# lab-incert/peba1

Hardware: AMD Instinct MI355X
Metric: bootstrapped gates/sec (blind rotations/s) over the PEBA1 match path, and end-to-end match ms (higher is better)
Workload: dtype u32

## Files before the change

include/tfhe_hip.h:

```cpp
#ifndef TFHE_HIP_H
#define TFHE_HIP_H

#include "tfhe/tfhe_core.h"

#ifdef __cplusplus
extern "C" {
#endif

enum TfheHipGate {
    TFHE_HIP_NAND = 0, TFHE_HIP_OR, TFHE_HIP_AND, TFHE_HIP_NOR, TFHE_HIP_XOR, TFHE_HIP_XNOR,
    TFHE_HIP_ANDNY, TFHE_HIP_ANDYN, TFHE_HIP_ORNY, TFHE_HIP_ORYN
};

const char *tfhe_hip_last_error(void);
void tfhe_hip_clear_error(void);

int tfhe_hip_set_device(int device);
int tfhe_hip_get_device(void);
int tfhe_hip_device_pci_bus_id(char *out, int len);

TFheGateBootstrappingParameterSet *tfhe_hip_new_parameters(
    int32_t n, int32_t N, int32_t k, int32_t l, int32_t Bgbit, int32_t ks_t, int32_t ks_basebit,
    double ks_stdev, double bk_stdev, double max_stdev);
TFheGateBootstrappingParameterSet *tfhe_hip_new_p2048_parameters(void);
// ... 103 lines not shown
    uint64_t clk_ref_ticks;
    uint64_t dead_gates;
    uint64_t folded_gates;
    uint64_t br_wide4_launches;
    uint64_t br_split_launches;
    uint64_t br_wave8_launches;
    uint64_t br_wave2_launches;
    uint64_t br_tables0_launches;
    uint64_t br_tables1_launches;
    uint64_t br_tables2_launches;
    uint64_t lut_rotations;
    uint64_t multi_rotations;
    uint64_t multi_outputs;
    uint64_t lincomb_ops;
    uint64_t lincomb_launches;
} TfheHipStats;
void tfhe_hip_get_stats(TfheHipStats *out);
void tfhe_hip_reset_stats(void);
void tfhe_hip_set_kernel_timing(int on);
int tfhe_hip_last_flush_keys(void);
int tfhe_hip_set_batch_keys(int on);

int tfhe_hip_test_form_admissible(int form, int32_t N, int32_t l, int32_t Bgbit, int tables);

void tfhe_hip_test_set_alloc_cap(int64_t bytes);

int tfhe_hip_test_schedule(const int32_t *ops5, int32_t count, int32_t unit, int32_t balance, int32_t *levels_out);
int tfhe_hip_test_level_plan(const int32_t *ops5, const int32_t *op_keys, int32_t count, int32_t nkeys, int32_t unit,
                             int32_t balance, int32_t *levels_out, int32_t *sizes6, int32_t *rot_off, int32_t *ks_off,
                             int32_t *rot_koff, int32_t *ks_koff, int32_t *rot_key, int32_t *rots6, int32_t *kss4);
// ... 2 lines not shown
                              int32_t *rot_koff, int32_t *ks_koff, int32_t *rot_key, int32_t *rots8, int32_t *kss4);
int tfhe_hip_test_level_plan_lut(const int32_t *ops10, const int32_t *op_keys, int32_t count, int32_t nkeys, int32_t unit,
                                 int32_t balance, int32_t reuse, int32_t *levels_out, int32_t *shared_with, int32_t *sizes6,
                                 int32_t *rot_off, int32_t *ks_off, int32_t *rot_koff, int32_t *ks_koff, int32_t *rot_key,
                                 int32_t *rots9, int32_t *kss4);
int tfhe_hip_test_level_plan_multi(const int32_t *ops16, const int32_t *op_keys, int32_t count, int32_t nkeys, int32_t unit,
                                   int32_t balance, int32_t reuse, const int32_t *dead_slots, int32_t ndead,
                                   int32_t *levels_out, int32_t *shared_with, int32_t *sizes6, int32_t *rot_off, int32_t *ks_off,
                                   int32_t *rot_koff, int32_t *ks_koff, int32_t *rot_key, int32_t *rots10, int32_t *kss4);
int tfhe_hip_test_level_plan_lin(const int32_t *ops16, const int32_t *op_keys, int32_t count, int32_t nkeys, int32_t unit,
                                 int32_t balance, int32_t reuse, const int32_t *dead_slots, int32_t ndead,
                                 const int32_t *lin_terms2, int32_t nterms, int32_t *levels_out, int32_t *ranks_out,
                                 int32_t *shared_with, int32_t *sizes6, int32_t *rot_off, int32_t *ks_off, int32_t *rot_koff,
                                 int32_t *ks_koff, int32_t *rot_key, int32_t *rots10, int32_t *kss4, int32_t *lin_sizes2,
                                 int32_t *lin_level_off, int32_t *lin_launch_off, int32_t *lin_launch_rank, int32_t *lins35);
int tfhe_hip_test_br_plan(int32_t N, int32_t l, int32_t Bgbit, const int32_t *tunings4, int32_t cu_count, int32_t count,
                          int32_t flags, int32_t *out3);
int tfhe_hip_test_ks_plan(int32_t n, int32_t N, int32_t k, int32_t ks_t, int32_t ks_basebit, const int32_t *tunings5,
                          int32_t cu_count, int32_t count, int64_t *out6);
int tfhe_hip_test_wg_times(const TFheGateBootstrappingCloudKeySet *bk, int32_t width, uint64_t *times4, double *launch_ms);

int tfhe_hip_kernel_negacyclic(const TFheGateBootstrappingCloudKeySet *bk, const int32_t *ip,
                               const Torus32 *tp, Torus32 *res, int32_t count);
int tfhe_hip_kernel_bootstrap_woks(const TFheGateBootstrappingCloudKeySet *bk, const Torus32 *lin,
                                   int32_t count, Torus32 *u_out, Torus32 *acc_out);
int tfhe_hip_kernel_lut_bootstrap_woks(const TFheGateBootstrappingCloudKeySet *bk, const Torus32 *lin, int32_t count,
                                       const int32_t *lut_index, const Torus32 *polys, int32_t npolys, Torus32 *u_out,
                                       Torus32 *acc_out);
#define TFHE_HIP_EXTRACT_SPEC_WORDS 73
int tfhe_hip_kernel_lut_bootstrap_multi_woks(const TFheGateBootstrappingCloudKeySet *bk, const Torus32 *lin, int32_t count,
// ... 11 lines not shown
```

peba1_amd/api.py:

```python
import ctypes as C

import numpy as np

from . import lib as _l

GATE_CODES = {"NAND": 0, "OR": 1, "AND": 2, "NOR": 3, "XOR": 4, "XNOR": 5,
              "ANDNY": 6, "ANDYN": 7, "ORNY": 8, "ORYN": 9}
GATE3_CODES = {"MAJ3": 0, "XOR3": 1, "XNOR3": 2}
GATE3_LIN = {"MAJ3": 1, "XOR3": -2, "XNOR3": 2}


def _i32p(a):
    assert a.dtype == np.int32 and a.flags["C_CONTIGUOUS"]
    return a.ctypes.data_as(_l.I32P)


def last_error():
    return _l.load().tfhe_hip_last_error().decode()


class _CFile:
    _libc = None

    def __init__(self, path, mode):
# ... 398 lines not shown

def flush_async():
    return _l.load().tfhe_hip_flush_async()


def wait():
    return _l.load().tfhe_hip_wait()


def set_tuning(name, value):
    if _l.load().tfhe_hip_set_tuning(name.encode(), int(value)) != 0:
        raise ValueError(last_error())


def stats():
    s = _l.StatsAll()
    _l.load().tfhe_hip_get_stats(C.byref(s))
    return {f: getattr(s, f) for f in _l.STATS_FIELDS}


def last_flush_keys():
    return _l.load().tfhe_hip_last_flush_keys()


def reset_stats():
    _l.load().tfhe_hip_reset_stats()


def kernel_negacyclic(key, ip, tp):
    ip = np.ascontiguousarray(ip, dtype=np.int32)
    tp = np.ascontiguousarray(tp, dtype=np.int32)
    res = np.zeros_like(tp)
    rc = _l.load().tfhe_hip_kernel_negacyclic(key.cloud, _i32p(ip), _i32p(tp), _i32p(res), ip.shape[0])
# ... 73 lines not shown
```

peba1_amd/csrc/engine.cpp:

```cpp
#include "engine.hpp"

#include <algorithm>
#include <utility>
#include <vector>
#include <chrono>
#include <ctime>
#include <unistd.h>
#include <cstdio>
#include <cstdlib>
#include <cstring>
#include <mutex>

#include "br_forms.hpp"
#include "ntt_field.hpp"

namespace tfhe_hip {

static std::string g_last_error;
static std::mutex g_err_mtx;

void set_error(const std::string &msg) {
    std::lock_guard<std::mutex> g(g_err_mtx);
    g_last_error = msg;
}
// ... 73 lines not shown
    for (size_t i = new_cap; i-- > cap_;) free_.push_back((int32_t)i);
    cap_ = new_cap;
}
int32_t SlotPool::alloc() {
    if (free_.empty()) {
        if (cap_ >= max_cap_)
            api_fail("ciphertext slot pool exhausted (" + std::to_string(max_cap_) +
                     " slots); raise TFHE_HIP_POOL_SLOTS or free ciphertext arrays");
        grow(std::min(max_cap_, cap_ * 2));
    }
    const int32_t s = free_.back();
    free_.pop_back();
    ref_[s] = 1;
    level[s] = 0;
    pending[s] = 0;
    return s;
}
void SlotPool::release(int32_t s) {
    if (s < 0) return;
    if (--ref_[s] == 0) free_.push_back(s);
}

Engine &Engine::get() {
    static Engine e;
    return e;
}

void Engine::set_device(int d) {
    if (inited_.load() && d != device_) fatal("tfhe_hip_set_device after the engine was initialised");
    device_ = d;
// ... 316 lines not shown
    if (n_ring < 1 || n_ring > LUT_STRIDE) api_fail("a test polynomial of more than " + std::to_string(LUT_STRIDE) + " words");
    return g_luts.add(pad_rows(words, 1, (size_t)n_ring, LUT_STRIDE).data());
}
void Engine::lut_free(int32_t index) { g_luts.release(index); }

int32_t Engine::spec_add(const ExtractSpec &xs) {
    ENGINE_DEVICE_SCOPE();
    ensure_init();
    if (g_specs.free.empty() && g_specs.used == g_specs.cap && g_specs.cap > (size_t)XS_ENTRY_MASK / 2) api_fail("too many extract specs");
    const int32_t index = g_specs.add(&xs);
    if (spec_nout_.size() <= (size_t)index) spec_nout_.resize((size_t)index + 1, 0);
    spec_nout_[(size_t)index] = xs.nout;
    return index;
}
void Engine::spec_free(int32_t index) { g_specs.release(index); }

SlotPool *Engine::find_pool(const Params &p) const {
    for (SlotPool *pl : pools_)
        if (pl->ct_stride() == p.ct_stride() && pl->ct_words() == p.ct_words()) return pl;
    return nullptr;
}

SlotPool *Engine::pool_for(const Params &p) {
    ENGINE_DEVICE_SCOPE();
    ensure_init();
    if (SlotPool *pl = find_pool(p)) return pl;
    size_t cap = 1u << 22;
    if (const char *env = std::getenv("TFHE_HIP_POOL_SLOTS")) cap = (size_t)std::atoll(env);
    if (cap < 8 || cap > MAX_POOL_SLOTS) {
        set_error("TFHE_HIP_POOL_SLOTS out of range [8, 2^29]; clamped");
// ... 539 lines not shown
```

peba1_amd/csrc/engine.hpp:

```cpp
#pragma once
#include <hip/hip_runtime.h>

#include <atomic>
#include <chrono>
#include <cstdint>
#include <string>
#include <vector>

#include "host_keys.hpp"
#include "br_forms.hpp"
#include "launch_plan.hpp"
#include "kernels.hpp"
#include "../../include/tfhe_hip.h"

struct DeviceKeyImage {
    tfhe_hip::DevParams dp;
    tfhe_hip::DevKey key;
    bool form_ok[tfhe_hip::BR_FORM_COUNT][3] = {};
    uint32_t *bk_img = nullptr;
    int32_t *ksk = nullptr;
    uint32_t *tw = nullptr;
    size_t bk_img_bytes = 0, ksk_bytes = 0, tw_bytes = 0;
};

// ... 13 lines not shown

class SlotPool {
public:
    SlotPool(int ct_words, int ct_stride, size_t capacity);
    ~SlotPool();
    int32_t alloc();
    void retain(int32_t s) { ++ref_[s]; }
    int32_t refs(int32_t s) const { return ref_[s]; }
    void release(int32_t s);
    int32_t *data() { return data_; }
    int ct_stride() const { return stride_; }
    int ct_words() const { return words_; }
    size_t capacity() const { return max_cap_; }
    size_t allocated() const { return cap_; }
    size_t in_use() const { return cap_ - free_.size(); }
    std::vector<int32_t> level;
    std::vector<uint8_t> pending;
    int32_t const_slot[2] = {-1, -1};
private:
    void grow(size_t new_cap);
    int words_, stride_;
    size_t cap_ = 0, max_cap_;
    int32_t *data_ = nullptr;
    std::vector<int32_t> ref_;
    std::vector<int32_t> free_;
};

struct LevelPlan {
    std::vector<RotDesc> rots;
    std::vector<KsDesc> kss;
    std::vector<NotDesc> nots;
    int levels = 0;
    std::vector<int32_t> rot_off, ks_off;
    std::vector<int32_t> not_off;
    std::vector<LinDesc> lins;
    std::vector<int32_t> lin_level_off, lin_launch_off, lin_launch_rank, op_rank;
    int32_t max_rots = 0;
// ... 4 lines not shown
    std::vector<tfhe_hip::DevKey> dev_keys;
};

class Engine {
public:
    static Engine &get();
    void ensure_init();
    int device() const { return device_; }
    int cu_count() const { return cu_count_; }
    void set_device(int d);
    hipStream_t stream() const { return stream_; }

    DeviceKeyImage *upload_key(const TfheHipCloudKey &ck);
    void free_key(DeviceKeyImage *img);
    SlotPool *pool_for(const Params &p);
    SlotPool *find_pool(const Params &p) const;

    void write_slot(SlotPool *pool, int32_t slot, const Torus32 *a, Torus32 b);
    void read_slot(SlotPool *pool, int32_t slot, Torus32 *a, Torus32 *b);
    void write_slots_packed(SlotPool *pool, const int32_t *slots, int count, const Torus32 *words, bool words_on_device, bool wait = true);
    void read_slots_packed(SlotPool *pool, const int32_t *slots, int count, Torus32 *words, bool words_on_device, bool wait = true);

    void execute(const std::vector<const DeviceKeyImage *> &keys, SlotPool *pool, LevelPlan &&plan, bool wait = true);
    int last_flush_keys = 0;
    void wait_flight();
    void sync_stream(const char *what);
    void sync_io();
    void wait_all() { wait_flight(); sync_io(); }
    void wait_event(hipEvent_t ev, const char *what, long long deadline_ms, const std::string &label);
    bool pci_bus_id(char *out, int len);
// ... 92 lines not shown
```

peba1_amd/csrc/op_graph.hpp:

```cpp
#pragma once
#include <algorithm>
#include <cstdint>
#include <unordered_map>
#include <unordered_set>
#include <vector>

#include "scheduler.hpp"

namespace tfhe_hip {

template <class Slots>
class OpGraph {
public:
    bool reuse = true;

    const std::vector<PendingOp> &ops() const { return ops_; }
    int32_t max_level() const { return max_level_; }
    const LinTerm *terms() const { return terms_.data(); }
    size_t term_count() const { return terms_.size(); }
    int32_t not_origin(int32_t slot) const {
        auto it = not_origin_.find(slot);
        return it == not_origin_.end() ? -1 : it->second;
    }

// ... 88 lines not shown
        int32_t depth = 0;
        for (size_t i = 0; i < ops_.size(); ++i) {
            if (at[i] < 0) continue;
            depth = std::max(depth, ops_[i].level);
            if (w != i) ops_[w] = ops_[i];
            at[i] = (int32_t)w++;
        }
        ops_.resize(w);
        max_level_ = depth;
        if (dead)
            for (auto &entry : index_) entry.second = at[(size_t)entry.second];
        if (moved_to) moved_to->swap(at);
        return dead;
    }

    void clear(std::vector<PendingOp> *into = nullptr, std::vector<LinTerm> *terms_into = nullptr) {
        if (into) into->swap(ops_);
        if (terms_into) terms_into->swap(terms_);
        ops_.clear();
        terms_.clear();
        index_.clear();
        not_origin_.clear();
        lin_dst_.clear();
        max_level_ = 0;
    }

private:
    std::vector<PendingOp> ops_;
    int32_t max_level_ = 0;
    std::unordered_map<OpKey, int32_t, OpKeyHash> index_;
// ... 7 lines not shown
```

peba1_amd/csrc/recorder.cpp:

```cpp
#include "recorder.hpp"

#include <algorithm>
#include <cstdio>
#include <cstdlib>
#include <cstring>
#include <utility>
#include <vector>

#include "op_graph.hpp"

namespace tfhe_hip {
namespace {

const uint8_t GATE_TT[10][4] = {
    {1, 1, 1, 0}, {0, 1, 1, 1}, {0, 0, 0, 1}, {1, 0, 0, 0}, {0, 1, 1, 0}, {1, 0, 0, 1},
    {0, 1, 0, 0}, {0, 0, 1, 0}, {1, 1, 0, 1}, {1, 0, 1, 1},
};

struct Recorder {
    std::recursive_mutex mtx;
    bool deferred = true;
    std::vector<const TFheGateBootstrappingCloudKeySet *> keys;
    uint16_t cur_key = 0;
    SlotPool *pool = nullptr;
    bool batch_keys = false;
    OpGraph<SlotPool> graph;
    bool balance_levels = true;
    std::vector<PendingOp> flight_ops;
    std::vector<LinTerm> flight_terms;
    SlotPool *flight_pool = nullptr;
    std::vector<const TFheGateBootstrappingCloudKeySet *> flight_keys;
    bool eliminate_dead = true;
    bool fold_constants = false;
};
Recorder &rec() {
    static Recorder r;
    static bool init = [] {
        if (const char *e = std::getenv("TFHE_HIP_DEFERRED")) r.deferred = std::atoi(e) != 0;
        if (const char *e = std::getenv("TFHE_HIP_FOLD_CONSTANTS")) r.fold_constants = std::atoi(e) != 0;
        if (const char *e = std::getenv("TFHE_HIP_BATCH_KEYS")) r.batch_keys = std::atoi(e) != 0;
        return true;
    }();
    (void)init;
    return r;
}

void release_refs(SlotPool *pool, const PendingOp &op, const LinTerm *terms) {
    for_each_src(op, terms, [&](int32_t s) { pool->release(s); });
    for_each_dst(op, [&](int32_t d) { pool->release(d); });
}

bool same_evaluation_params(const Params &a, const Params &b) {
    return a.n == b.n && a.N == b.N && a.k == b.k && a.l == b.l && a.Bgbit == b.Bgbit && a.ks_t == b.ks_t &&
           a.ks_basebit == b.ks_basebit;
}
// ... 304 lines not shown
    if (const char *trace = std::getenv("TFHE_HIP_TRACE_DAG")) {
        if (FILE *f = std::fopen(trace, "w")) {
            for (size_t i = 0; i < ops.size(); ++i)
                std::fprintf(f, "%d %d %d %d %d %d %d %d\n", (int)ops[i].kind, ops[i].level, alap[i], lvl[i],
                             ops[i].dst, ops[i].a, ops[i].b, ops[i].c);
            std::fclose(f);
        }
    }
    std::vector<int32_t> remap(r.keys.size(), -1);
    for (const PendingOp &op : ops) remap[op.key] = 0;
    std::vector<const TFheGateBootstrappingCloudKeySet *> used;
    std::vector<const DeviceKeyImage *> images;
    for (size_t k = 0; k < r.keys.size(); ++k)
        if (remap[k] == 0) { remap[k] = (int32_t)used.size(); used.push_back(r.keys[k]); images.push_back(r.keys[k]->bk->dev); }
    LevelPlan plan;
    if (used.size() == r.keys.size()) {
        plan = build_level_plan(ops, lvl, levels, (int)used.size(), r.graph.terms());
    } else {
        std::vector<PendingOp> rekeyed = ops;
        for (PendingOp &op : rekeyed) op.key = (uint16_t)remap[op.key];
        plan = build_level_plan(rekeyed, lvl, levels, (int)used.size(), r.graph.terms());
    }
    finish_flight_locked();
    Engine::get().execute(images, pool, std::move(plan), wait);
    for (const PendingOp &op : ops) {
        for_each_dst(op, [&](int32_t d) {
            pool->level[d] = 0;
            pool->pending[d] = 0;
        });
        if (wait) release_refs(pool, op, r.graph.terms());
    }
    if (!wait) { r.flight_pool = pool; r.flight_keys = std::move(used); }
    r.graph.clear(wait ? nullptr : &r.flight_ops, wait ? nullptr : &r.flight_terms);
    return levels;
}

void flush_pending_locked(bool wait) { if (!rec().graph.ops().empty()) flush_locked(wait); }

void forget_key_locked(const TFheGateBootstrappingCloudKeySet *bk) {
// ... 4 lines not shown
}

bool deferred_mode() { return rec().deferred; }

bool set_deferred_locked(bool on) { return std::exchange(rec().deferred, on); }

bool set_batch_keys_locked(bool on) { return std::exchange(rec().batch_keys, on); }

bool set_recorder_tuning_locked(const char *name, bool on) {
    Recorder &r = rec();
    bool *knob = std::strcmp(name, "reuse_gates") == 0      ? &r.graph.reuse
                 : std::strcmp(name, "eliminate_dead") == 0 ? &r.eliminate_dead
                 : std::strcmp(name, "fold_constants") == 0 ? &r.fold_constants
                 : std::strcmp(name, "balance_levels") == 0 ? &r.balance_levels
                 : std::strcmp(name, "batch_keys") == 0     ? &r.batch_keys
                                                            : nullptr;
    if (knob) *knob = on;
    return knob != nullptr;
}

}
```

peba1_amd/csrc/scheduler.cpp:

```cpp
#include "scheduler.hpp"

#include "engine.hpp"

#include <algorithm>
#include <queue>
#include <unordered_map>

namespace tfhe_hip {

namespace {
struct HeapItem {
    int32_t alap, idx;
    bool operator>(const HeapItem &o) const { return alap != o.alap ? alap > o.alap : idx > o.idx; }
};
}


int schedule_levels(const std::vector<PendingOp> &ops, int asap_depth, bool balance, int unit,
                    std::vector<int32_t> &lvl, std::vector<int32_t> *alap_out, const LinTerm *terms) {
    const int n = (int)ops.size();
    lvl.resize(n);
    for (int i = 0; i < n; ++i) lvl[i] = ops[i].level;
    if (alap_out) *alap_out = lvl;
    if (!balance || asap_depth <= 2 || n < 4 * unit) return asap_depth;
// ... 135 lines not shown
        const PendingOp &op = ops[(size_t)order[j].second];
        LinDesc &d = plan.lins[j];
        d = LinDesc{};
        d.dst_slot = op.dst; d.nin = op.nout; d.c0 = op.c0;
        for (int t = 0; t < op.nout; ++t) { d.slot[t] = terms[op.spec + t].slot; d.coef[t] = terms[op.spec + t].coef; }
        if (j > 0 && order[j].first != order[j - 1].first) plan.lin_launch_off.push_back((int32_t)j);
        if (j == 0 || order[j].first != order[j - 1].first) {
            plan.lin_launch_rank.push_back((int32_t)(order[j].first & 0xFFFFFFFF));
            ++plan.lin_level_off[(size_t)(order[j].first >> 32) + 1];
        }
    }
    plan.lin_launch_off.push_back((int32_t)nlin);
    for (size_t L = 0; L <= (size_t)levels; ++L) plan.lin_level_off[L + 1] += plan.lin_level_off[L];
}

LevelPlan build_level_plan(const std::vector<PendingOp> &ops, const std::vector<int32_t> &lvl, int levels, int nkeys,
                           const LinTerm *terms) {
    LevelPlan plan;
    plan.levels = levels;
    plan.nkeys = nkeys;
    plan_linear_ops(plan, ops, lvl, levels, terms);
    const size_t groups = (size_t)levels * nkeys;
    std::vector<int32_t> roff(groups + 1, 0), koff(groups + 1, 0), uoff(groups + 1, 0);
    plan.not_off.assign((size_t)levels + 2, 0);
    for (size_t i = 0; i < ops.size(); ++i) {
        if (ops[i].kind == OP_NOT) { ++plan.not_off[(size_t)lvl[i] + 1]; continue; }
        if (ops[i].kind == OP_LIN) continue;
        const size_t sg = (size_t)(lvl[i] - 1) * nkeys + ops[i].key;
        roff[sg + 1] += op_rotations(ops[i]);
        koff[sg + 1] += op_keyswitches(ops[i]);
        uoff[sg + 1] += op_extracts(ops[i]);
    }
// ... 72 lines not shown
```

peba1_amd/csrc/scheduler.hpp:

```cpp
#pragma once
#include <cstddef>
#include <cstdint>
#include <utility>
#include <vector>

namespace tfhe_hip {

struct PendingOp {
    uint8_t kind;
    int32_t dst, a, b, c;
    int32_t level;
    uint16_t key = 0;
    int32_t lut = -1;
    int32_t sa = 0, sb = 0, sc = 0, c0 = 0;
    int32_t spec = -1;
    int32_t nout = 0;
    int32_t dsts[4] = {-1, -1, -1, -1};
};
constexpr uint8_t OP_MUX = 16, OP_NOT = 17;
constexpr uint8_t OP_LUT = 64;
constexpr uint8_t OP_GATE3 = 32, OP_GATE3_END = OP_GATE3 + 3 * 8;
inline bool op_is_gate3(int kind) { return kind >= OP_GATE3 && kind < OP_GATE3_END; }
inline bool op_kind_valid(int kind) { return (kind >= 0 && kind < 10) || kind == OP_MUX || kind == OP_NOT || op_is_gate3(kind); }
inline bool op_kind_valid_lut(int kind) { return op_kind_valid(kind) || kind == OP_LUT; }
// ... 61 lines not shown
            h ^= ((uint64_t)(uint32_t)k.sa << 40 ^ (uint64_t)(uint32_t)k.sb << 20 ^ (uint32_t)k.sc) * 0xFF51AFD7ED558CCDull;
        }
        return (size_t)(h ^ (h >> 29));
    }
};
inline OpKey op_key(const PendingOp &op) {
    int32_t a = op.a, b = op.b;
    if (op.kind < OP_MUX && GATE_LIN[op.kind].sa == GATE_LIN[op.kind].sb && b < a) std::swap(a, b);
    if (op.kind != OP_LUT && op.kind != OP_LUTM) return OpKey{op.kind, a, b, op.c, op.key, -1, 0, 0, 0, 0};
    return OpKey{op.kind, a, b, op.c, op.key, op.lut, op.sa, op.sb, op.sc, op.c0, op.kind == OP_LUTM ? op.spec : -1};
}

int schedule_levels(const std::vector<PendingOp> &ops, int asap_depth, bool balance, int unit,
                    std::vector<int32_t> &lvl, std::vector<int32_t> *alap_out = nullptr, const LinTerm *terms = nullptr);

struct LevelPlan;
__attribute__((visibility("hidden"))) LevelPlan build_level_plan(const std::vector<PendingOp> &ops,
                                                                 const std::vector<int32_t> &lvl, int levels, int nkeys = 1,
                                                                 const LinTerm *terms = nullptr);

}
```

peba1_amd/csrc/shim.cpp:

```cpp
#include <cstddef>
#include <cstdio>
#include <cstdlib>
#include <cstring>
#include <algorithm>
#include <numeric>
#include <string>
#include <vector>

#include "br_forms.hpp"
#include "engine.hpp"
#include "op_graph.hpp"
#include "recorder.hpp"
#include "scheduler.hpp"
#include "../../include/tfhe/tfhe.h"

using namespace tfhe_hip;

namespace tfhe_hip {
const std::string &last_error_ref();
bool io_forget_owned_cloud(const void *ks);
bool io_forget_owned_secret(const void *ks);
}

namespace {
// ... 844 lines not shown
    }
    if (name && std::strcmp(name, "ks_index") == 0) { Engine::get().tunings.ks_index = value != 0; return 0; }
    if (name && std::strcmp(name, "br_digit_table") == 0) { Engine::get().tunings.br_digit_table = (int)value; return 0; }
    if (name && std::strcmp(name, "br8_max_rotations") == 0) { Engine::get().tunings.br8_max_rotations = (int)value; return 0; }
    if (name && std::strcmp(name, "br_tail8") == 0) { Engine::get().tunings.br_tail8 = (int)value; return 0; }
    if (name && std::strcmp(name, "br_variant") == 0) { Engine::get().tunings.br_variant = (int)value; return 0; }
    if (name && set_recorder_tuning_locked(name, value != 0)) return 0;
    if (name && std::strcmp(name, "sync_deadline_ms") == 0) { Engine::get().sync_deadline_ms = value > 0 ? (long long)value : 0; return 0; }
    set_error(std::string("tfhe_hip_set_tuning: unknown name ") + (name ? name : "(null)"));
    return -1;
}

void tfhe_hip_get_stats(TfheHipStats *out) {
    auto g = recorder_lock();
    Engine::get().wait_flight();
    if (out) *out = Engine::get().stats;
}
void tfhe_hip_reset_stats(void) {
    auto g = recorder_lock();
    Engine::get().stats = TfheHipStats{};
}
void tfhe_hip_set_kernel_timing(int on) { Engine::get().kernel_timing = on != 0; }
int tfhe_hip_last_flush_keys(void) {
    auto g = recorder_lock();
    return Engine::get().last_flush_keys;
}
int tfhe_hip_set_batch_keys(int on) {
    auto g = recorder_lock();
    return set_batch_keys_locked(on != 0) ? 1 : 0;
}

static int test_build_ops(const int32_t *ops5, int32_t count, std::vector<PendingOp> &ops) {
    for (int32_t i = 0; i < count; ++i)
        if (!op_kind_valid(ops5[5 * (size_t)i])) { set_error("test schedule: unknown op kind"); return -1; }
    ops.resize((size_t)count);
// ... 14 lines not shown
}

int tfhe_hip_test_schedule(const int32_t *ops5, int32_t count, int32_t unit, int32_t balance, int32_t *levels_out) {
    std::vector<PendingOp> ops;
    const int depth = test_build_ops(ops5, count, ops);
    if (depth < 0) return -1;
    std::vector<int32_t> lvl;
    const int d = schedule_levels(ops, depth, balance != 0, unit, lvl);
    for (int32_t i = 0; i < count; ++i) levels_out[i] = lvl[i];
    return d;
}

struct TestLinPlan {
    const int32_t *terms2; int32_t nterms;
    int32_t *ranks_out, *sizes2, *level_off, *launch_off, *launch_rank, *descs35;
};
static int test_level_plan(const int32_t *ops5, const int32_t *op_keys, int32_t count, int32_t nkeys, int32_t unit,
                           int32_t balance, int32_t *levels_out, int32_t *sizes6, int32_t *rot_off, int32_t *ks_off,
                           int32_t *rot_koff, int32_t *ks_koff, int32_t *rot_key, int32_t *rots, int rot_words, int32_t *kss4,
                           bool lut_ops = false, int32_t reuse = 0, int32_t *shared_with = nullptr, int rec_words = 10,
                           const int32_t *dead_slots = nullptr, int32_t ndead = 0, const TestLinPlan *lin = nullptr) {
    if (count < 0 || nkeys < 1 || nkeys > UINT16_MAX) { set_error("test_level_plan: bad count or nkeys"); return -1; }
    for (int32_t i = 0; i < count; ++i)
        if (op_keys[i] < 0 || op_keys[i] >= nkeys) { set_error("test_level_plan: key index out of range"); return -1; }
    std::vector<PendingOp> ops;
    std::vector<int32_t> op_of_record;
    std::vector<LinTerm> terms;
    int depth;
    if (!lut_ops) {
        depth = test_build_ops(ops5, count, ops);
        if (depth < 0) return -1;
        for (int32_t i = 0; i < count; ++i) ops[i].key = (uint16_t)op_keys[i];
    } else {
        struct SlotTable {
            std::vector<int32_t> ref, level;
            std::vector<uint8_t> pending;
            void retain(int32_t s) { ++ref[(size_t)s]; }
            void release(int32_t s) { --ref[(size_t)s]; }
            int32_t refs(int32_t s) const { return ref[(size_t)s]; }
        };
        const int id_words = rec_words == 16 ? 4 : 0;
        int32_t top = 0;
// ... 50 lines not shown
            if (shared_with) shared_with[i] = shared < 0 ? -1 : record_of_op[(size_t)shared];
            op_of_record[(size_t)i] = shared < 0 ? (int32_t)record_of_op.size() - 1 : shared;
            for (int m = 0; m < op_outputs(op); ++m)
                if ((wanted >> m & 1) && out[m] != ids[m]) { slots.release(ids[m]); handle[(size_t)ids[m]] = out[m]; }
        }
        for (int32_t d = 0; d < ndead; ++d) {
            const int32_t id = dead_slots[d];
            if (id < 0 || id >= top || handle[(size_t)id] < 0) continue;
            slots.release(handle[(size_t)id]);
            handle[(size_t)id] = -1;
        }
        std::vector<int32_t> moved_to;
        graph.eliminate_dead(slots, &moved_to);
        for (int32_t &at : op_of_record) at = moved_to[(size_t)at];
        ops = graph.ops();
        terms.assign(graph.terms(), graph.terms() + graph.term_count());
        depth = graph.max_level();
    }
    std::vector<int32_t> lvl;
    const int levels = schedule_levels(ops, depth, balance != 0, unit, lvl, nullptr, terms.data());
    const LevelPlan plan = build_level_plan(ops, lvl, levels, nkeys, terms.data());
    for (int32_t i = 0; i < count; ++i) {
        const int32_t at = lut_ops ? op_of_record[(size_t)i] : i;
        levels_out[i] = at >= 0 ? lvl[(size_t)at] : -1;
        if (lin) lin->ranks_out[i] = at < 0 ? -1 : plan.op_rank.empty() ? 0 : plan.op_rank[(size_t)at];
    }
    if (lin) {
        static_assert(sizeof(LinDesc) == 35 * sizeof(int32_t), "a linear descriptor is 35 plain words");
        lin->sizes2[0] = plan.lins.empty() ? 0 : (int32_t)plan.lin_launch_off.size() - 1;
        lin->sizes2[1] = (int32_t)plan.lins.size();
        for (size_t L = 0; L < (size_t)levels + 2; ++L) lin->level_off[L] = plan.lins.empty() ? 0 : plan.lin_level_off[L];
        if (!plan.lins.empty()) {
            std::memcpy(lin->launch_off, plan.lin_launch_off.data(), plan.lin_launch_off.size() * sizeof(int32_t));
            std::memcpy(lin->launch_rank, plan.lin_launch_rank.data(), plan.lin_launch_rank.size() * sizeof(int32_t));
            std::memcpy(lin->descs35, plan.lins.data(), plan.lins.size() * sizeof(LinDesc));
        }
// ... 56 lines not shown
                                 const int32_t *lin_terms2, int32_t nterms, int32_t *levels_out, int32_t *ranks_out,
                                 int32_t *shared_with, int32_t *sizes6, int32_t *rot_off, int32_t *ks_off, int32_t *rot_koff,
                                 int32_t *ks_koff, int32_t *rot_key, int32_t *rots10, int32_t *kss4, int32_t *lin_sizes2,
                                 int32_t *lin_level_off, int32_t *lin_launch_off, int32_t *lin_launch_rank, int32_t *lins35) {
    if (!shared_with || !ranks_out || !lin_sizes2 || !lin_level_off || !lin_launch_off || !lin_launch_rank || !lins35) {
        set_error("test_level_plan_lin: null output");
        return -1;
    }
    if (ndead < 0 || (ndead > 0 && !dead_slots)) { set_error("test_level_plan_lin: bad dead_slots"); return -1; }
    if (nterms < 0 || (nterms > 0 && !lin_terms2)) { set_error("test_level_plan_lin: bad term table"); return -1; }
    const TestLinPlan lin{lin_terms2, nterms, ranks_out, lin_sizes2, lin_level_off, lin_launch_off, lin_launch_rank, lins35};
    return test_level_plan(ops16, op_keys, count, nkeys, unit, balance, levels_out, sizes6, rot_off, ks_off, rot_koff, ks_koff,
                           rot_key, rots10, 10, kss4, true, reuse, shared_with, 16, dead_slots, ndead, &lin);
}

int tfhe_hip_test_br_plan(int32_t N, int32_t l, int32_t Bgbit, const int32_t *tunings4, int32_t cu_count, int32_t count,
                          int32_t flags, int32_t *out3) {
    if (!tunings4 || !out3 || cu_count < 1 || count < 1) { set_error("test_br_plan: bad arguments"); return -1; }
    LaunchTunings t;
    t.br_variant = tunings4[0]; t.br8_max_rotations = tunings4[1]; t.br_tail8 = tunings4[2]; t.br_digit_table = tunings4[3];
    bool form_ok[BR_FORM_COUNT][3];
    fill_form_ok(form_ok, N, l, Bgbit);
    const BrPlan plan = plan_br(form_ok, N, l, t, cu_count, count, (flags & 1) != 0, (flags & 2) != 0);
    out3[0] = plan.form; out3[1] = plan.tables; out3[2] = plan.tail;
    return 0;
}

int tfhe_hip_test_ks_plan(int32_t n, int32_t N, int32_t k, int32_t ks_t, int32_t ks_basebit, const int32_t *tunings5,
                          int32_t cu_count, int32_t count, int64_t *out6) {
    if (!tunings5 || !out6 || cu_count < 1 || count < 1) { set_error("test_ks_plan: bad arguments"); return -1; }
// ... 83 lines not shown
```

peba1_amd/lib.py:

```python
import ctypes as C
import os

_HERE = os.path.dirname(os.path.abspath(__file__))
LIB_PATH = os.environ.get("PEBA1_TFHE_HIP_LIB") or os.path.join(_HERE, "libtfhe-hip.so")
CIRCUITS_PATH = os.path.join(_HERE, "libpeba1-circuits.so")


class LweSample(C.Structure):
    _fields_ = [("a", C.POINTER(C.c_int32)), ("b", C.c_int32), ("slot", C.c_int32),
                ("current_variance", C.c_double)]


class LweParams(C.Structure):
    _fields_ = [("n", C.c_int32), ("alpha_min", C.c_double), ("alpha_max", C.c_double)]


class TLweParams(C.Structure):
    _fields_ = [("N", C.c_int32), ("k", C.c_int32), ("alpha_min", C.c_double), ("alpha_max", C.c_double)]


class TGswParams(C.Structure):
    _fields_ = [("l", C.c_int32), ("Bgbit", C.c_int32), ("Bg", C.c_int32), ("halfBg", C.c_int32),
                ("maskMod", C.c_uint32), ("tlwe_params", C.POINTER(TLweParams)), ("kpl", C.c_int32),
                ("offset", C.c_uint32)]
# ... 21 lines not shown
                ("br8_launches", C.c_uint64), ("br8_rotations", C.c_uint64), ("ms_blind_rotate8", C.c_double),
                ("clk_shader_cycles", C.c_uint64), ("clk_ref_ticks", C.c_uint64), ("dead_gates", C.c_uint64),
                ("folded_gates", C.c_uint64),
                ("br_wide4_launches", C.c_uint64), ("br_split_launches", C.c_uint64),
                ("br_wave8_launches", C.c_uint64), ("br_wave2_launches", C.c_uint64),
                ("br_tables0_launches", C.c_uint64), ("br_tables1_launches", C.c_uint64),
                ("br_tables2_launches", C.c_uint64), ("lut_rotations", C.c_uint64),
                ("multi_rotations", C.c_uint64), ("multi_outputs", C.c_uint64)]


class StatsAll(Stats):
    _fields_ = [("lincomb_ops", C.c_uint64), ("lincomb_launches", C.c_uint64)]


STATS_FIELDS = [f for f, _ in Stats._fields_] + [f for f, _ in StatsAll._fields_]


PS = C.POINTER(ParameterSet)
CK = C.POINTER(CloudKeySet)
SK = C.POINTER(SecretKeySet)
LS = C.POINTER(LweSample)
I32P = C.POINTER(C.c_int32)

_GATE2 = ["bootsAND", "bootsOR", "bootsXOR", "bootsXNOR", "bootsNAND", "bootsNOR", "bootsANDNY", "bootsANDYN",
          "bootsORNY", "bootsORYN"]
SIGNATURES = {
    "new_gate_bootstrapping_ciphertext_array": (LS, [C.c_int32, PS]),
    "delete_gate_bootstrapping_ciphertext_array": (None, [C.c_int32, LS]),
    "new_gate_bootstrapping_ciphertext": (LS, [PS]),
    "delete_gate_bootstrapping_ciphertext": (None, [LS]),
# ... 66 lines not shown
    "tfhe_hip_new_lut_multi_from_tables": (C.c_void_p, [PS, C.c_int32, C.c_int32, C.c_int32, I32P]),
    "tfhe_hip_delete_lut_multi": (None, [C.c_void_p]),
    "tfhe_hip_lut_multi_nout": (C.c_int32, [C.c_void_p]),
    "tfhe_hip_lut_multi_output": (C.c_int32, [C.c_void_p, C.c_int32, I32P, I32P, I32P]),
    "tfhe_hip_lut_multi_words": (I32P, [C.c_void_p, I32P]),
    "tfhe_hip_lut_bootstrap_multi": (None, [C.c_void_p, C.POINTER(LS), C.c_int32, C.POINTER(LS), I32P, C.c_int32, CK]),
    "tfhe_hip_lut_bootstrap_multi_batch": (C.c_int, [C.c_void_p, C.POINTER(LS), C.c_int32, C.POINTER(LS), I32P, C.c_int32,
                                                     C.c_int32, CK]),
    "tfhe_hip_linear": (None, [LS, C.c_int32, C.POINTER(LS), I32P, C.c_int32, CK]),
    "tfhe_hip_linear_batch": (C.c_int, [LS, C.c_int32, C.POINTER(LS), I32P, C.c_int32, C.c_int32, CK]),
    "tfhe_hip_sym_encrypt_torus": (None, [LS, C.c_int32, SK]),
    "tfhe_hip_sym_phase": (C.c_int32, [LS, SK]),
    "tfhe_hip_set_tuning": (C.c_int, [C.c_char_p, C.c_int64]),
    "tfhe_hip_test_form_admissible": (C.c_int, [C.c_int, C.c_int32, C.c_int32, C.c_int32, C.c_int]),
    "tfhe_hip_test_set_alloc_cap": (None, [C.c_int64]),
    "tfhe_hip_get_stats": (None, [C.POINTER(StatsAll)]),
    "tfhe_hip_reset_stats": (None, []),
    "tfhe_hip_set_kernel_timing": (None, [C.c_int]),
    "tfhe_hip_last_flush_keys": (C.c_int, []),
    "tfhe_hip_set_batch_keys": (C.c_int, [C.c_int]),
    "tfhe_hip_test_schedule": (C.c_int, [I32P, C.c_int32, C.c_int32, C.c_int32, I32P]),
    "tfhe_hip_test_level_plan": (C.c_int, [I32P, I32P, C.c_int32, C.c_int32, C.c_int32, C.c_int32] + [I32P] * 9),
    "tfhe_hip_test_level_plan3": (C.c_int, [I32P, I32P, C.c_int32, C.c_int32, C.c_int32, C.c_int32] + [I32P] * 9),
    "tfhe_hip_test_level_plan_lut": (C.c_int, [I32P, I32P, C.c_int32, C.c_int32, C.c_int32, C.c_int32, C.c_int32] + [I32P] * 10),
    "tfhe_hip_test_level_plan_multi": (C.c_int, [I32P, I32P, C.c_int32, C.c_int32, C.c_int32, C.c_int32, C.c_int32, I32P,
                                                 C.c_int32] + [I32P] * 10),
    "tfhe_hip_test_level_plan_lin": (C.c_int, [I32P, I32P, C.c_int32, C.c_int32, C.c_int32, C.c_int32, C.c_int32, I32P,
                                               C.c_int32, I32P, C.c_int32] + [I32P] * 16),
    "tfhe_hip_test_br_plan": (C.c_int, [C.c_int32] * 3 + [I32P, C.c_int32, C.c_int32, C.c_int32, I32P]),
    "tfhe_hip_test_ks_plan": (C.c_int, [C.c_int32] * 5 + [I32P, C.c_int32, C.c_int32, C.POINTER(C.c_int64)]),
    "tfhe_hip_kernel_negacyclic":(C.c_int, [CK, I32P, I32P, I32P, C.c_int32]),
    "tfhe_hip_kernel_bootstrap_woks": (C.c_int, [CK, I32P, C.c_int32, I32P, I32P]),
    "tfhe_hip_kernel_lut_bootstrap_woks": (C.c_int, [CK, I32P, C.c_int32, I32P, I32P, C.c_int32, I32P, I32P]),
    "tfhe_hip_kernel_lut_bootstrap_multi_woks": (C.c_int, [CK, I32P, C.c_int32, I32P, I32P, C.c_int32, I32P, I32P, C.c_int32,
                                                           I32P, I32P]),
    "tfhe_hip_kernel_keyswitch": (C.c_int, [CK, I32P, C.c_int32, I32P]),
}
for _g in _GATE2:
    SIGNATURES[_g] = (None, [LS, LS, LS, CK])
_lib = None


def load():
# ... 15 lines not shown
```

Before: 108,100.

## Rename temporary ciphertext slots to reuse dead slots within a flush

```diff
diff --git a/include/tfhe_hip.h b/include/tfhe_hip.h
--- a/include/tfhe_hip.h
+++ b/include/tfhe_hip.h
@@ -141,6 +141,8 @@
     uint64_t multi_outputs;
     uint64_t lincomb_ops;
     uint64_t lincomb_launches;
+    uint64_t reused_slots;
+    uint64_t pool_high_water;
 } TfheHipStats;
 void tfhe_hip_get_stats(TfheHipStats *out);
 void tfhe_hip_reset_stats(void);
@@ -173,6 +175,13 @@
                                  int32_t *shared_with, int32_t *sizes6, int32_t *rot_off, int32_t *ks_off, int32_t *rot_koff,
                                  int32_t *ks_koff, int32_t *rot_key, int32_t *rots10, int32_t *kss4, int32_t *lin_sizes2,
                                  int32_t *lin_level_off, int32_t *lin_launch_off, int32_t *lin_launch_rank, int32_t *lins35);
+int tfhe_hip_test_level_plan_reuse(const int32_t *ops16, const int32_t *op_keys, int32_t count, int32_t nkeys, int32_t unit,
+                                   int32_t balance, int32_t reuse, const int32_t *dead_slots, int32_t ndead,
+                                   const int32_t *lin_terms2, int32_t nterms, int32_t reuse_slots, int32_t *slot_of,
+                                   int32_t nslot_of, int32_t *reused_out, int32_t *levels_out, int32_t *ranks_out,
+                                   int32_t *shared_with, int32_t *sizes6, int32_t *rot_off, int32_t *ks_off, int32_t *rot_koff,
+                                   int32_t *ks_koff, int32_t *rot_key, int32_t *rots10, int32_t *kss4, int32_t *lin_sizes2,
+                                   int32_t *lin_level_off, int32_t *lin_launch_off, int32_t *lin_launch_rank, int32_t *lins35);
 int tfhe_hip_test_br_plan(int32_t N, int32_t l, int32_t Bgbit, const int32_t *tunings4, int32_t cu_count, int32_t count,
                           int32_t flags, int32_t *out3);
 int tfhe_hip_test_ks_plan(int32_t n, int32_t N, int32_t k, int32_t ks_t, int32_t ks_basebit, const int32_t *tunings5,
diff --git a/peba1_amd/api.py b/peba1_amd/api.py
--- a/peba1_amd/api.py
+++ b/peba1_amd/api.py
@@ -436,9 +436,15 @@
 
 
 def stats():
-    s = _l.StatsAll()
+    s = _l.StatsPool()
     _l.load().tfhe_hip_get_stats(C.byref(s))
     return {f: getattr(s, f) for f in _l.STATS_FIELDS}
+
+
+def pool_stats():
+    s = _l.StatsPool()
+    _l.load().tfhe_hip_get_stats(C.byref(s))
+    return {f: getattr(s, f) for f in _l.POOL_STATS_FIELDS}
 
 
 def last_flush_keys():
diff --git a/peba1_amd/csrc/engine.cpp b/peba1_amd/csrc/engine.cpp
--- a/peba1_amd/csrc/engine.cpp
+++ b/peba1_amd/csrc/engine.cpp
@@ -111,6 +111,7 @@
     ref_[s] = 1;
     level[s] = 0;
     pending[s] = 0;
+    high_water_ = std::max(high_water_, in_use());
     return s;
 }
 void SlotPool::release(int32_t s) {
@@ -457,6 +458,15 @@
     return index;
 }
 void Engine::spec_free(int32_t index) { g_specs.release(index); }
+
+size_t Engine::pool_high_water(bool reset) {
+    size_t most = 0;
+    for (SlotPool *pl : pools_) {
+        if (reset) pl->reset_high_water();
+        most = std::max(most, pl->high_water());
+    }
+    return most;
+}
 
 SlotPool *Engine::find_pool(const Params &p) const {
     for (SlotPool *pl : pools_)
diff --git a/peba1_amd/csrc/engine.hpp b/peba1_amd/csrc/engine.hpp
--- a/peba1_amd/csrc/engine.hpp
+++ b/peba1_amd/csrc/engine.hpp
@@ -51,13 +51,15 @@
     size_t capacity() const { return max_cap_; }
     size_t allocated() const { return cap_; }
     size_t in_use() const { return cap_ - free_.size(); }
+    size_t high_water() const { return high_water_; }
+    void reset_high_water() { high_water_ = in_use(); }
     std::vector<int32_t> level;
     std::vector<uint8_t> pending;
     int32_t const_slot[2] = {-1, -1};
 private:
     void grow(size_t new_cap);
     int words_, stride_;
-    size_t cap_ = 0, max_cap_;
+    size_t cap_ = 0, max_cap_, high_water_ = 0;
     int32_t *data_ = nullptr;
     std::vector<int32_t> ref_;
     std::vector<int32_t> free_;
@@ -92,6 +94,7 @@
     DeviceKeyImage *upload_key(const TfheHipCloudKey &ck);
     void free_key(DeviceKeyImage *img);
     SlotPool *pool_for(const Params &p);
+    size_t pool_high_water(bool reset = false);
     SlotPool *find_pool(const Params &p) const;
 
     void write_slot(SlotPool *pool, int32_t slot, const Torus32 *a, Torus32 b);
diff --git a/peba1_amd/csrc/op_graph.hpp b/peba1_amd/csrc/op_graph.hpp
--- a/peba1_amd/csrc/op_graph.hpp
+++ b/peba1_amd/csrc/op_graph.hpp
@@ -126,6 +126,17 @@
         return dead;
     }
 
+    std::vector<int32_t> temporaries(const Slots &slots) const {
+        int32_t max_slot = -1;
+        for (const PendingOp &op : ops_) for_each_dst(op, [&](int32_t d) { max_slot = std::max(max_slot, d); });
+        std::vector<int32_t> readers((size_t)max_slot + 1, 0), out;
+        for (const PendingOp &op : ops_)
+            for_each_src(op, terms_.data(), [&](int32_t s) { if (s <= max_slot) ++readers[(size_t)s]; });
+        for (const PendingOp &op : ops_)
+            for_each_dst(op, [&](int32_t d) { if (slots.refs(d) == 1 + readers[(size_t)d]) out.push_back(d); });
+        return out;
+    }
+
     void clear(std::vector<PendingOp> *into = nullptr, std::vector<LinTerm> *terms_into = nullptr) {
         if (into) into->swap(ops_);
         if (terms_into) terms_into->swap(terms_);
diff --git a/peba1_amd/csrc/recorder.cpp b/peba1_amd/csrc/recorder.cpp
--- a/peba1_amd/csrc/recorder.cpp
+++ b/peba1_amd/csrc/recorder.cpp
@@ -32,6 +32,7 @@
     std::vector<const TFheGateBootstrappingCloudKeySet *> flight_keys;
     bool eliminate_dead = true;
     bool fold_constants = false;
+    bool reuse_slots = true;
 };
 Recorder &rec() {
     static Recorder r;
@@ -39,6 +40,7 @@
         if (const char *e = std::getenv("TFHE_HIP_DEFERRED")) r.deferred = std::atoi(e) != 0;
         if (const char *e = std::getenv("TFHE_HIP_FOLD_CONSTANTS")) r.fold_constants = std::atoi(e) != 0;
         if (const char *e = std::getenv("TFHE_HIP_BATCH_KEYS")) r.batch_keys = std::atoi(e) != 0;
+        if (const char *e = std::getenv("TFHE_HIP_REUSE_SLOTS")) r.reuse_slots = std::atoi(e) != 0;
         return true;
     }();
     (void)init;
@@ -373,15 +375,19 @@
     for (size_t k = 0; k < r.keys.size(); ++k)
         if (remap[k] == 0) { remap[k] = (int32_t)used.size(); used.push_back(r.keys[k]); images.push_back(r.keys[k]->bk->dev); }
     LevelPlan plan;
+    SlotReuse slot_reuse;
+    if (r.reuse_slots) slot_reuse.temporaries = r.graph.temporaries(*pool);
+    SlotReuse *const renaming = r.reuse_slots ? &slot_reuse : nullptr;
     if (used.size() == r.keys.size()) {
-        plan = build_level_plan(ops, lvl, levels, (int)used.size(), r.graph.terms());
+        plan = build_level_plan(ops, lvl, levels, (int)used.size(), r.graph.terms(), renaming);
     } else {
         std::vector<PendingOp> rekeyed = ops;
         for (PendingOp &op : rekeyed) op.key = (uint16_t)remap[op.key];
-        plan = build_level_plan(rekeyed, lvl, levels, (int)used.size(), r.graph.terms());
+        plan = build_level_plan(rekeyed, lvl, levels, (int)used.size(), r.graph.terms(), renaming);
     }
     finish_flight_locked();
     Engine::get().execute(images, pool, std::move(plan), wait);
+    Engine::get().stats.reused_slots += slot_reuse.reused;
     for (const PendingOp &op : ops) {
         for_each_dst(op, [&](int32_t d) {
             pool->level[d] = 0;
@@ -416,6 +422,7 @@
                  : std::strcmp(name, "fold_constants") == 0 ? &r.fold_constants
                  : std::strcmp(name, "balance_levels") == 0 ? &r.balance_levels
                  : std::strcmp(name, "batch_keys") == 0     ? &r.batch_keys
+                 : std::strcmp(name, "reuse_slots") == 0    ? &r.reuse_slots
                                                             : nullptr;
     if (knob) *knob = on;
     return knob != nullptr;
diff --git a/peba1_amd/csrc/scheduler.cpp b/peba1_amd/csrc/scheduler.cpp
--- a/peba1_amd/csrc/scheduler.cpp
+++ b/peba1_amd/csrc/scheduler.cpp
@@ -173,8 +173,66 @@
     for (size_t L = 0; L <= (size_t)levels; ++L) plan.lin_level_off[L + 1] += plan.lin_level_off[L];
 }
 
+static void plan_slot_reuse(SlotReuse &reuse, const std::vector<PendingOp> &ops, const std::vector<int32_t> &lvl, int levels,
+                            const LinTerm *terms) {
+    reuse.reused = 0;
+    reuse.renamed.clear();
+    if (reuse.temporaries.empty()) return;
+    const int32_t max_slot = *std::max_element(reuse.temporaries.begin(), reuse.temporaries.end());
+    std::vector<int32_t> last((size_t)max_slot + 1, -1);
+    for (const int32_t s : reuse.temporaries) last[(size_t)s] = 0;
+    auto temporary = [&](int32_t s) { return s <= max_slot && last[(size_t)s] >= 0; };
+    std::vector<int32_t> at((size_t)levels + 2, 0), order(ops.size());
+    for (size_t i = 0; i < ops.size(); ++i) {
+        ++at[(size_t)lvl[i] + 1];
+        auto use = [&](int32_t s) { if (temporary(s)) last[(size_t)s] = std::max(last[(size_t)s], lvl[i]); };
+        for_each_src(ops[i], terms, use);
+        for_each_dst(ops[i], use);
+    }
+    for (size_t L = 0; L <= (size_t)levels; ++L) at[L + 1] += at[L];
+    {
+        std::vector<int32_t> cursor(at.begin(), at.end() - 1);
+        for (size_t i = 0; i < ops.size(); ++i) order[(size_t)cursor[(size_t)lvl[i]]++] = (int32_t)i;
+    }
+    reuse.renamed.assign((size_t)max_slot + 1, -1);
+    std::vector<int32_t> free;
+    std::vector<std::vector<int32_t>> dies((size_t)levels + 1);
+    for (int L = 0; L <= levels; ++L) {
+        if (L > 0) free.insert(free.end(), dies[(size_t)L - 1].begin(), dies[(size_t)L - 1].end());
+        for (int32_t j = at[(size_t)L]; j < at[(size_t)L + 1]; ++j)
+            for_each_dst(ops[(size_t)order[(size_t)j]], [&](int32_t d) {
+                if (!temporary(d)) return;
+                int32_t home = d;
+                if (!free.empty()) {
+                    home = free.back();
+                    free.pop_back();
+                    reuse.renamed[(size_t)d] = home;
+                    ++reuse.reused;
+                }
+                dies[(size_t)last[(size_t)d]].push_back(home);
+            });
+    }
+}
+
+static void rename_slots(LevelPlan &plan, const std::vector<int32_t> &renamed) {
+    auto fix = [&](int32_t &s) { if (s >= 0 && (size_t)s < renamed.size() && renamed[(size_t)s] >= 0) s = renamed[(size_t)s]; };
+    for (RotDesc &r : plan.rots) { fix(r.slot_a); fix(r.slot_b); fix(r.slot_c); }
+    for (KsDesc &k : plan.kss) fix(k.dst_slot);
+    for (NotDesc &n : plan.nots) { fix(n.src_slot); fix(n.dst_slot); }
+    for (LinDesc &d : plan.lins) {
+        fix(d.dst_slot);
+        for (int t = 0; t < d.nin; ++t) fix(d.slot[t]);
+    }
+}
+
 LevelPlan build_level_plan(const std::vector<PendingOp> &ops, const std::vector<int32_t> &lvl, int levels, int nkeys,
-                           const LinTerm *terms) {
+                           const LinTerm *terms, SlotReuse *reuse) {
+    if (reuse) {
+        plan_slot_reuse(*reuse, ops, lvl, levels, terms);
+        LevelPlan plan = build_level_plan(ops, lvl, levels, nkeys, terms, nullptr);
+        if (reuse->reused) rename_slots(plan, reuse->renamed);
+        return plan;
+    }
     LevelPlan plan;
     plan.levels = levels;
     plan.nkeys = nkeys;
diff --git a/peba1_amd/csrc/scheduler.hpp b/peba1_amd/csrc/scheduler.hpp
--- a/peba1_amd/csrc/scheduler.hpp
+++ b/peba1_amd/csrc/scheduler.hpp
@@ -99,9 +99,14 @@
 int schedule_levels(const std::vector<PendingOp> &ops, int asap_depth, bool balance, int unit,
                     std::vector<int32_t> &lvl, std::vector<int32_t> *alap_out = nullptr, const LinTerm *terms = nullptr);
 
+struct SlotReuse {
+    std::vector<int32_t> temporaries;
+    std::vector<int32_t> renamed;
+    size_t reused = 0;
+};
 struct LevelPlan;
 __attribute__((visibility("hidden"))) LevelPlan build_level_plan(const std::vector<PendingOp> &ops,
                                                                  const std::vector<int32_t> &lvl, int levels, int nkeys = 1,
-                                                                 const LinTerm *terms = nullptr);
+                                                                 const LinTerm *terms = nullptr, SlotReuse *reuse = nullptr);
 
 }
diff --git a/peba1_amd/csrc/shim.cpp b/peba1_amd/csrc/shim.cpp
--- a/peba1_amd/csrc/shim.cpp
+++ b/peba1_amd/csrc/shim.cpp
@@ -882,11 +882,13 @@
 void tfhe_hip_get_stats(TfheHipStats *out) {
     auto g = recorder_lock();
     Engine::get().wait_flight();
+    Engine::get().stats.pool_high_water = Engine::get().pool_high_water();
     if (out) *out = Engine::get().stats;
 }
 void tfhe_hip_reset_stats(void) {
     auto g = recorder_lock();
     Engine::get().stats = TfheHipStats{};
+    (void)Engine::get().pool_high_water(true);
 }
 void tfhe_hip_set_kernel_timing(int on) { Engine::get().kernel_timing = on != 0; }
 int tfhe_hip_last_flush_keys(void) {
@@ -931,6 +933,7 @@
 struct TestLinPlan {
     const int32_t *terms2; int32_t nterms;
     int32_t *ranks_out, *sizes2, *level_off, *launch_off, *launch_rank, *descs35;
+    int32_t reuse_slots = 0; int32_t *slot_of = nullptr; int32_t nslot_of = 0; int32_t *reused = nullptr;
 };
 static int test_level_plan(const int32_t *ops5, const int32_t *op_keys, int32_t count, int32_t nkeys, int32_t unit,
                            int32_t balance, int32_t *levels_out, int32_t *sizes6, int32_t *rot_off, int32_t *ks_off,
@@ -943,6 +946,7 @@
     std::vector<PendingOp> ops;
     std::vector<int32_t> op_of_record;
     std::vector<LinTerm> terms;
+    std::vector<int32_t> temporaries;
     int depth;
     if (!lut_ops) {
         depth = test_build_ops(ops5, count, ops);
@@ -1023,12 +1027,21 @@
         graph.eliminate_dead(slots, &moved_to);
         for (int32_t &at : op_of_record) at = moved_to[(size_t)at];
         ops = graph.ops();
+        if (lin && lin->reuse_slots) temporaries = graph.temporaries(slots);
         terms.assign(graph.terms(), graph.terms() + graph.term_count());
         depth = graph.max_level();
     }
     std::vector<int32_t> lvl;
     const int levels = schedule_levels(ops, depth, balance != 0, unit, lvl, nullptr, terms.data());
-    const LevelPlan plan = build_level_plan(ops, lvl, levels, nkeys, terms.data());
+    SlotReuse slot_reuse;
+    if (lin && lin->reuse_slots) slot_reuse.temporaries.swap(temporaries);
+    const LevelPlan plan = build_level_plan(ops, lvl, levels, nkeys, terms.data(),
+                                            lin && lin->reuse_slots ? &slot_reuse : nullptr);
+    if (lin && lin->slot_of) {
+        for (int32_t s = 0; s < lin->nslot_of; ++s)
+            lin->slot_of[s] = (size_t)s < slot_reuse.renamed.size() && slot_reuse.renamed[(size_t)s] >= 0 ? slot_reuse.renamed[(size_t)s] : s;
+        *lin->reused = (int32_t)slot_reuse.reused;
+    }
     for (int32_t i = 0; i < count; ++i) {
         const int32_t at = lut_ops ? op_of_record[(size_t)i] : i;
         levels_out[i] = at >= 0 ? lvl[(size_t)at] : -1;
@@ -1115,6 +1128,26 @@
                            rot_key, rots10, 10, kss4, true, reuse, shared_with, 16, dead_slots, ndead, &lin);
 }
 
+int tfhe_hip_test_level_plan_reuse(const int32_t *ops16, const int32_t *op_keys, int32_t count, int32_t nkeys, int32_t unit,
+                                   int32_t balance, int32_t reuse, const int32_t *dead_slots, int32_t ndead,
+                                   const int32_t *lin_terms2, int32_t nterms, int32_t reuse_slots, int32_t *slot_of,
+                                   int32_t nslot_of, int32_t *reused_out, int32_t *levels_out, int32_t *ranks_out,
+                                   int32_t *shared_with, int32_t *sizes6, int32_t *rot_off, int32_t *ks_off, int32_t *rot_koff,
+                                   int32_t *ks_koff, int32_t *rot_key, int32_t *rots10, int32_t *kss4, int32_t *lin_sizes2,
+                                   int32_t *lin_level_off, int32_t *lin_launch_off, int32_t *lin_launch_rank, int32_t *lins35) {
+    if (!shared_with || !ranks_out || !lin_sizes2 || !lin_level_off || !lin_launch_off || !lin_launch_rank || !lins35 ||
+        !slot_of || !reused_out || nslot_of < 0) {
+        set_error("test_level_plan_reuse: null output");
+        return -1;
+    }
+    if (ndead < 0 || (ndead > 0 && !dead_slots)) { set_error("test_level_plan_reuse: bad dead_slots"); return -1; }
+    if (nterms < 0 || (nterms > 0 && !lin_terms2)) { set_error("test_level_plan_reuse: bad term table"); return -1; }
+    TestLinPlan lin{lin_terms2, nterms, ranks_out, lin_sizes2, lin_level_off, lin_launch_off, lin_launch_rank, lins35};
+    lin.reuse_slots = reuse_slots; lin.slot_of = slot_of; lin.nslot_of = nslot_of; lin.reused = reused_out;
+    return test_level_plan(ops16, op_keys, count, nkeys, unit, balance, levels_out, sizes6, rot_off, ks_off, rot_koff, ks_koff,
+                           rot_key, rots10, 10, kss4, true, reuse, shared_with, 16, dead_slots, ndead, &lin);
+}
+
 int tfhe_hip_test_br_plan(int32_t N, int32_t l, int32_t Bgbit, const int32_t *tunings4, int32_t cu_count, int32_t count,
                           int32_t flags, int32_t *out3) {
     if (!tunings4 || !out3 || cu_count < 1 || count < 1) { set_error("test_br_plan: bad arguments"); return -1; }
diff --git a/peba1_amd/lib.py b/peba1_amd/lib.py
--- a/peba1_amd/lib.py
+++ b/peba1_amd/lib.py
@@ -59,6 +59,13 @@
 
 
 STATS_FIELDS = [f for f, _ in Stats._fields_] + [f for f, _ in StatsAll._fields_]
+
+
+class StatsPool(StatsAll):
+    _fields_ = [("reused_slots", C.c_uint64), ("pool_high_water", C.c_uint64)]
+
+
+POOL_STATS_FIELDS = [f for f, _ in StatsPool._fields_]
 
 
 PS = C.POINTER(ParameterSet)
@@ -155,7 +162,7 @@
     "tfhe_hip_set_tuning": (C.c_int, [C.c_char_p, C.c_int64]),
     "tfhe_hip_test_form_admissible": (C.c_int, [C.c_int, C.c_int32, C.c_int32, C.c_int32, C.c_int]),
     "tfhe_hip_test_set_alloc_cap": (None, [C.c_int64]),
-    "tfhe_hip_get_stats": (None, [C.POINTER(StatsAll)]),
+    "tfhe_hip_get_stats": (None, [C.POINTER(StatsPool)]),
     "tfhe_hip_reset_stats": (None, []),
     "tfhe_hip_set_kernel_timing": (None, [C.c_int]),
     "tfhe_hip_last_flush_keys": (C.c_int, []),
@@ -168,6 +175,8 @@
                                                  C.c_int32] + [I32P] * 10),
     "tfhe_hip_test_level_plan_lin": (C.c_int, [I32P, I32P, C.c_int32, C.c_int32, C.c_int32, C.c_int32, C.c_int32, I32P,
                                                C.c_int32, I32P, C.c_int32] + [I32P] * 16),
+    "tfhe_hip_test_level_plan_reuse": (C.c_int, [I32P, I32P, C.c_int32, C.c_int32, C.c_int32, C.c_int32, C.c_int32, I32P,
+                                                 C.c_int32, I32P, C.c_int32, C.c_int32, I32P, C.c_int32, I32P] + [I32P] * 16),
     "tfhe_hip_test_br_plan": (C.c_int, [C.c_int32] * 3 + [I32P, C.c_int32, C.c_int32, C.c_int32, I32P]),
     "tfhe_hip_test_ks_plan": (C.c_int, [C.c_int32] * 5 + [I32P, C.c_int32, C.c_int32, C.POINTER(C.c_int64)]),
     "tfhe_hip_kernel_negacyclic":(C.c_int, [CK, I32P, I32P, I32P, C.c_int32]),
```

Result: no change. 108,100 (median of 2 runs) (-0.1%).
